# gMedAI-Lab/GAViKO

Hardware: AMD Instinct MI355X
Metric: MRI volumes/sec (fwd+bwd) ViT-B/16 gaviko, 120x160x160 (higher is better)
Workload: dtype bf16

## Files before the change

gaviko_amd/csrc/gemm_bf16.hip:

```cpp
#include "gemm_epilogue.hpp"

namespace gvk {

template <int BK>
__device__ __forceinline__ int swz_chunk(int row) {
  if constexpr (BK == 64) return (row >> 1) & 7;
  else return (0x78 >> (((row >> 2) & 3) * 2)) & 3;
}

template <int BM, int BN, int EPI, int BK = 64, bool DROP = false, int NS = 2, int NW = 4, bool SPLITK = false>
__global__ __launch_bounds__(64 * NW) void gemm_nt_kernel(GemmArgs p) {
  static_assert(NW == 4 || NW == 8, "4 or 8 waves");
  static_assert(!SPLITK || (NW == 4 && !DROP), "split-K is built on the 4-wave loops");
  static_assert(BK == 64, "the interleaved weight-row mapping is built for 128-byte tile rows");
  static_assert(NS >= 2 && NS <= 4, "2..4 LDS stages");
  constexpr int WM = BM / (NW / 2), WN = BN / 2;
  constexpr int MT = WM / 16, NT = WN / 16;
  constexpr int ROWB = BK * 2;
  constexpr int RPI = 1024 / ROWB;
  constexpr int CPR = ROWB / 16;
  constexpr int A_BYTES = BM * ROWB, W_BYTES = BN * ROWB, STAGE = A_BYTES + W_BYTES;
  extern __shared__ __attribute__((aligned(16))) char smem[];

  const int nwg = p.nbm * p.nbn;
// ... 29 lines not shown
  const bf16* __restrict__ Ag = p.A + (size_t)m0 * p.lda;
  const bf16* __restrict__ Wg = p.W + (size_t)n0 * p.ldw;
  if constexpr (SPLITK) {
    Ag += (size_t)piece * p.kt_per * BK;
    Wg += (size_t)piece * p.kt_per * BK;
  }

  auto stage = [&](int buf, int kt) {
    char* sA = smem + buf * STAGE;
    char* sW = sA + A_BYTES;
    const int k0 = kt * BK;
    const int rsub = lane / CPR, slot = lane % CPR;
#pragma unroll
    for (int r = 0; r < BM / (NW * RPI); ++r) {
      const int row = (r * NW + wave) * RPI + rsub;
      const int chunk = slot ^ swz_chunk<BK>(row);
      int srow = row;
      if constexpr (BM > 128 || 128 % BM != 0) srow = min(row, p.a_rows - 1 - m0);
      glds16(Ag + (size_t)srow * p.lda + k0 + chunk * 8, sA + (r * NW + wave) * 1024);
    }
#pragma unroll
    for (int r = 0; r < BN / (NW * RPI); ++r) {
      const int row = (r * NW + wave) * RPI + rsub;
      const int chunk = slot ^ swz_w(row);
      glds16(Wg + (size_t)row * p.ldw + k0 + chunk * 8, sW + (r * NW + wave) * 1024);
    }
  };

  f32x4 acc[MT][NT];
#pragma unroll
  for (int i = 0; i < MT; ++i)
#pragma unroll
    for (int j = 0; j < NT; ++j) acc[i][j] = f32x4{0.f, 0.f, 0.f, 0.f};

  int nt = p.K / BK;
  if constexpr (SPLITK) nt = min(p.kt_per, nt - piece * p.kt_per);
  if constexpr (BK == 64) {
#define GVK_LOAD_FRAGS(SA, SW, KS, XA, WB)                                                                  \
  {                                                                                                         \
    const int chunk_ = (KS) * 4 + lq;                                                                       \
    _Pragma("unroll") for (int i = 0; i < MT; ++i) {                                                        \
      const int row = wm * WM + i * 16 + l15;                                                               \
      XA[i] = *(const bf16x8*)((SA) + row * ROWB + ((chunk_ ^ swz_chunk<BK>(row)) << 4));                   \
    }                                                                                                       \
    _Pragma("unroll") for (int j = 0; j < NT; ++j) {                                                        \
      const int row = wn * WN + 32 * (j >> 1) + 8 * (l15 >> 2) + 4 * (j & 1) + (l15 & 3);                   \
      WB[j] = *(const bf16x8*)((SW) + row * ROWB + ((chunk_ ^ swz_w(row)) << 4));                           \
    }                                                                                                       \
  }
#define GVK_MMA(XA, WB)                                                                                      \
  _Pragma("unroll") for (int i = 0; i < MT; ++i)                                                            \
  _Pragma("unroll") for (int j = 0; j < NT; ++j)                                                            \
      acc[i][j] = __builtin_amdgcn_mfma_f32_16x16x32_bf16(WB[j], XA[i], acc[i][j], 0, 0, 0);
    bf16x8 xa0[MT], wb0[NT], xa1[MT], wb1[NT];
    constexpr int PER_TILE = BM / (NW * RPI) + BN / (NW * RPI);
    if constexpr (NS == 2) {
    stage(0, 0);
    if (nt > 1) stage(1, 1);
    if (nt > 1) __builtin_amdgcn_s_waitcnt(0x0F70 | (PER_TILE & 0xF) | ((PER_TILE >> 4) << 14));
    else __builtin_amdgcn_s_waitcnt(0x0F70);
    __builtin_amdgcn_s_barrier();
    GVK_LOAD_FRAGS(smem, smem + A_BYTES, 0, xa0, wb0)
    __builtin_amdgcn_s_waitcnt(0xC07F);
#define GVK_TILE(T, PREFETCH)                                                                               \
    {                                                                                                       \
      const int buf = (T) & 1;                                                                              \
      const char* sA = smem + buf * STAGE;                                                                  \
      const char* sW = sA + A_BYTES;                                                                        \
      GVK_LOAD_FRAGS(sA, sW, 1, xa1, wb1)                                                                   \
      __builtin_amdgcn_sched_barrier(0);                                                                    \
      GVK_MMA(xa0, wb0)                                                                                     \
      __builtin_amdgcn_sched_barrier(0);                                                                    \
      __syncthreads();     \
      if (PREFETCH) stage(buf, (T) + 2);                                                                    \
      GVK_LOAD_FRAGS(smem + (buf ^ 1) * STAGE, smem + (buf ^ 1) * STAGE + A_BYTES, 0, xa0, wb0)             \
      __builtin_amdgcn_sched_barrier(0);                                                                    \
      GVK_MMA(xa1, wb1)                                                                                     \
      __builtin_amdgcn_sched_barrier(0);                                                                    \
      __builtin_amdgcn_s_waitcnt(0xC07F);     \
    }
    int t = 0;
    for (; t < nt - 2; ++t) GVK_TILE(t, true)
    for (; t < nt; ++t) GVK_TILE(t, false)
#undef GVK_TILE
    } else {
    static_assert((NS - 1) * PER_TILE <= 63, "vmcnt is a 6-bit counter");
#pragma unroll
    for (int sgi = 0; sgi < NS; ++sgi)
      if (sgi < nt) stage(sgi, sgi);
    {
      const int ahead = min(nt, NS) - 1;
      if (ahead >= 3) __builtin_amdgcn_s_waitcnt(0x0F70 | ((3 * PER_TILE) & 0xF) | (((3 * PER_TILE) >> 4) << 14));
      else if (ahead == 2) __builtin_amdgcn_s_waitcnt(0x0F70 | ((2 * PER_TILE) & 0xF) | (((2 * PER_TILE) >> 4) << 14));
      else if (ahead == 1) __builtin_amdgcn_s_waitcnt(0x0F70 | (PER_TILE & 0xF) | ((PER_TILE >> 4) << 14));
      else __builtin_amdgcn_s_waitcnt(0x0F70);
    }
    __builtin_amdgcn_s_barrier();
    GVK_LOAD_FRAGS(smem, smem + A_BYTES, 0, xa0, wb0)
    __builtin_amdgcn_s_waitcnt(0xC07F);
#define GVK_TILE3(T, BUF, PREFETCH, AHEAD, LAST)                                                            \
    {                                                                                                       \
      const int buf = (BUF);                                                                                \
      const int nxt = buf == NS - 1 ? 0 : buf + 1;                                                          \
      const char* sA = smem + buf * STAGE;                                                                  \
      const char* sW = sA + A_BYTES;                                                                        \
      GVK_LOAD_FRAGS(sA, sW, 1, xa1, wb1)                                                                   \
      __builtin_amdgcn_sched_barrier(0);                                                                    \
      GVK_MMA(xa0, wb0)                                                                                     \
      __builtin_amdgcn_sched_barrier(0);                                                                    \
       \
      __builtin_amdgcn_s_waitcnt(0x0070 | (((AHEAD) * PER_TILE) & 0xF) | ((((AHEAD) * PER_TILE) >> 4) << 14)); \
      __builtin_amdgcn_s_barrier();                                                                         \
      if (PREFETCH) stage(buf, (T) + NS);                                                                   \
      if (!(LAST)) GVK_LOAD_FRAGS(smem + nxt * STAGE, smem + nxt * STAGE + A_BYTES, 0, xa0, wb0)            \
      __builtin_amdgcn_sched_barrier(0);                                                                    \
      GVK_MMA(xa1, wb1)                                                                                     \
      __builtin_amdgcn_sched_barrier(0);                                                                    \
      __builtin_amdgcn_s_waitcnt(0xC07F);                                                                   \
    }
    int t = 0, b = 0;
    for (; t < nt - NS; ++t) {
      GVK_TILE3(t, b, true, NS - 2, false)
      b = b == NS - 1 ? 0 : b + 1;
    }
    for (; t < nt; ++t) {
      const int r = nt - 1 - t;
      if (NS > 3 && r == 3) GVK_TILE3(t, b, false, 2, false)
      else if (r == 2) GVK_TILE3(t, b, false, 1, false)
      else if (r == 1) GVK_TILE3(t, b, false, 0, false)
      else GVK_TILE3(t, b, false, 0, true)
      b = b == NS - 1 ? 0 : b + 1;
    }
#undef GVK_TILE3
    }
#undef GVK_LOAD_FRAGS
#undef GVK_MMA
  }

  if constexpr (SPLITK) {
    const int tile_id = tile_m * p.nbn + tile_n;
    constexpr int kPiece = NW * MT * NT * 64 * 4;
    float* const base = p.sk_part + ((size_t)tile_id * p.ksplit) * kPiece;
    const __amdgpu_buffer_rsrc_t rs = __builtin_amdgcn_make_buffer_rsrc((void*)base, 0, p.ksplit * kPiece * 4, 0x00020000);
    const int off = ((wave * MT * NT) * 64 + lane) * 16;
#pragma unroll
    for (int i = 0; i < MT; ++i)
#pragma unroll
      for (int j = 0; j < NT; ++j)
        __builtin_amdgcn_raw_buffer_store_b128(__builtin_bit_cast(u32x4, acc[i][j]), rs, (piece * kPiece) * 4 + off + (i * NT + j) * 1024, 0, 16);
    int* const s_last = (int*)smem;
    asm volatile("s_waitcnt vmcnt(0)" ::: "memory");
    __syncthreads();
    if (threadIdx.x == 0) {
      const int t = __hip_atomic_fetch_add(p.sk_tick + tile_id, 1, __ATOMIC_RELAXED, __HIP_MEMORY_SCOPE_AGENT);
      const int last = (t == p.ksplit - 1) ? 1 : 0;
      if (last) {
        __builtin_amdgcn_fence(__ATOMIC_ACQUIRE, "agent");
        asm volatile("s_waitcnt vmcnt(0)" ::: "memory");
        __hip_atomic_store(p.sk_tick + tile_id, 0, __ATOMIC_RELAXED, __HIP_MEMORY_SCOPE_AGENT);
      }
      *s_last = last;
    }
    __syncthreads();
    if (!*s_last) return;
    if (p.ksplit == 2) {
      const int pc = piece ^ 1;
#pragma unroll
      for (int i = 0; i < MT; ++i)
#pragma unroll
        for (int j = 0; j < NT; ++j) acc[i][j] += *(const f32x4*)((const char*)base + (size_t)pc * kPiece * 4 + off + (i * NT + j) * 1024);
    } else {
#pragma unroll
      for (int i = 0; i < MT; ++i)
#pragma unroll
        for (int j = 0; j < NT; ++j) acc[i][j] = f32x4{0.f, 0.f, 0.f, 0.f};
      for (int pc = 0; pc < p.ksplit; ++pc) {
#pragma unroll
        for (int i = 0; i < MT; ++i)
#pragma unroll
          for (int j = 0; j < NT; ++j) acc[i][j] += *(const f32x4*)((const char*)base + (size_t)pc * kPiece * 4 + off + (i * NT + j) * 1024);
      }
    }
  }
  gemm_epilogue<EPI, DROP, MT, NT>(p, acc, m0 + wm * WM, n0 + wn * WN, l15, lq);
}

template <int BM, int BN, int EPI, bool DROP = false, int NS = 2, int NW = 4, bool SPLITK = false>
static int launch_gemm(const GemmArgs& a, hipStream_t stream) {
  constexpr int BK = 64;
  constexpr int lds = NS * (BM + BN) * BK * 2;
  static bool attr_set = false;
  if (!attr_set) {
    hipError_t e = hipFuncSetAttribute(reinterpret_cast<const void*>(&gemm_nt_kernel<BM, BN, EPI, BK, DROP, NS, NW, SPLITK>),
                                       hipFuncAttributeMaxDynamicSharedMemorySize, lds);
    if (e != hipSuccess) return set_error(-3, "hipFuncSetAttribute(gemm %dx%d): %s", BM, BN, hipGetErrorString(e));
    attr_set = true;
  }
  GemmArgs p = a;
  p.nbm = (a.M + BM - 1) / BM;
  p.nbn = a.N / BN;
  p.a_rows = (a.M + 127) / 128 * 128;
  p.m_stride = BM;
  if (a.m_stride > 0) {
    if (a.m_stride < BM || (long)(a.nbm - 1) * a.m_stride + BM > p.a_rows)
      return set_error(-2, "gvk_gemm_nt_bf16: %d row panels of %d rows at stride %d do not fit %d (padded) rows", a.nbm, BM, a.m_stride, p.a_rows);
    p.nbm = a.nbm;
    p.m_stride = a.m_stride;
  }
  {
    const int per_xcd = (p.nbm * p.nbn) >> 3;
    int g = (per_xcd + p.nbn / 2) / p.nbn;
    g = g < 1 ? 1 : g > 8 ? 8 : g;
    static const int force = diag_env("GAVIKO_HIP_GEMM_GROUP_M") ? atoi(diag_env("GAVIKO_HIP_GEMM_GROUP_M")) : 0;
    p.group_m = force > 0 ? force : g;
  }
  const int grid = p.nbm * p.nbn;
  p.xcd_panels = 0;
  {
    static const int mode = diag_env("GAVIKO_HIP_GEMM_XCD_PANELS") ? atoi(diag_env("GAVIKO_HIP_GEMM_XCD_PANELS")) : 1;
    if (mode != 0 && NS >= 3 && grid <= 256) p.xcd_panels = 1;
  }
  if constexpr (SPLITK) {
    const int nt = a.K / BK;
    int s = 256 / (grid > 0 ? grid : 1);
    s = s < 1 ? 1 : s > 8 ? 8 : s;
    if (a.ksplit > 0) s = a.ksplit;
    if (s > nt / 2) s = nt / 2 > 0 ? nt / 2 : 1;
    p.kt_per = (nt + s - 1) / s;
    p.ksplit = (nt + p.kt_per - 1) / p.kt_per;
    constexpr size_t kPiece = (size_t)NW * (BM / (NW / 2) / 16) * (BN / 2 / 16) * 64 * 4 * 4;
    const size_t need = 1024 + (size_t)grid * p.ksplit * kPiece;
    if (a.sk_part == nullptr || a.sk_bytes < need || grid > 256)
      return set_error(-2, "gvk_gemm_nt_bf16: split-K workspace of %zu bytes needed (%zu given; at most 256 tiles)", need, a.sk_bytes);
    p.sk_tick = (int*)a.sk_part;
    p.sk_part = (float*)((char*)a.sk_part + 1024);
    GVK_LAUNCH((gemm_nt_kernel<BM, BN, EPI, BK, DROP, NS, NW, SPLITK>), dim3(grid * p.ksplit), dim3(64 * NW), lds, stream, p);
    return check_launch("gemm_nt_bf16 (split-K panels)");
  }
  GVK_LAUNCH((gemm_nt_kernel<BM, BN, EPI, BK, DROP, NS, NW, SPLITK>), dim3(grid), dim3(64 * NW), lds, stream, p);
  return check_launch("gemm_nt_bf16");
}

static long wide_lo() {
  static const long v = diag_env("GAVIKO_HIP_GEMM_WIDE_LO") ? atol(diag_env("GAVIKO_HIP_GEMM_WIDE_LO")) : 140;
  return v;
}

template <int EPI>
static int dispatch_tile(const GemmArgs& a, int tile, hipStream_t stream) {
  if (a.m_stride > 0) {
    if (tile == 0) tile = (a.N % 128 == 0 && a.drop_thresh == 0u) ? 4064128 : 64064;
    if (tile == 8256256 || tile == 7256256 || tile == 256256) return set_error(-2, "gvk_gemm_nt_bf16: strided row panels run on the 4-wave tiles only");
  }
  if (tile == 0) {
    const int bn = (a.N % 128 == 0) ? 128 : 64;
    const long t128 = (long)((a.M + 127) / 128) * (a.N / bn);
    static const int n768 = diag_env("GAVIKO_HIP_GEMM_N768") ? atoi(diag_env("GAVIKO_HIP_GEMM_N768")) : 3128;
    const int bm = (t128 >= 384) ? 128 : 64;
    tile = bm * 1000 + bn;
    if constexpr (EPI == GVK_EPI_STORE_BF16 || EPI == GVK_EPI_BIAS_GELU_BF16 || EPI == GVK_EPI_GELU_BWD_BF16) {
      static const int wide = diag_env("GAVIKO_HIP_GEMM_WIDE") ? atoi(diag_env("GAVIKO_HIP_GEMM_WIDE")) : 8;
      const long t256 = (long)((a.M + 255) / 256) * (a.N / 256);
      static const bool wide_bwd = diag_env("GAVIKO_HIP_GEMM_WIDE_BWD") == nullptr || diag_env("GAVIKO_HIP_GEMM_WIDE_BWD")[0] != '0';
      if (wide != 0 && a.N % 256 == 0 && a.drop_thresh == 0u && t256 >= wide_lo() && t256 <= 256 && (EPI != GVK_EPI_GELU_BWD_BF16 || wide_bwd))
        tile = (wide == 256 || a.K < 128) ? 256256 : 8256256;
    }
    static const long t64_hi = diag_env("GAVIKO_HIP_GEMM_T64HI") ? atol(diag_env("GAVIKO_HIP_GEMM_T64HI")) : 130;
    if (bm == 64 && bn == 128 && t128 <= 256 && a.K >= 512 && a.drop_thresh == 0u) {
      if (n768 == 3128) {
        long best = -1; int best_bm = 128;
        for (int cand : {128, 96, 64}) {
          const long tiles = (long)((a.M + cand - 1) / cand) * (a.N / 128);
          const long cost = ((tiles + 255) / 256) * (cand + 128);
          if (best < 0 || cost < best) { best = cost; best_bm = cand; }
        }
        static const int force_bm = diag_env("GAVIKO_HIP_GEMM_BM") ? atoi(diag_env("GAVIKO_HIP_GEMM_BM")) : 0;
        if (force_bm == 128 || force_bm == 96 || force_bm == 64) best_bm = force_bm;
        else if (t128 <= t64_hi && best_bm == 128) best_bm = 64;
        tile = best_bm == 64 ? 3064128 : best_bm == 96 ? 3096128 : 3128128;
      }
      else if (n768 == 128) tile = 128128;
      else if (n768 == 3064) tile = 3064128;
    }
  }
  if (a.drop_thresh != 0u) {
    if constexpr (EPI == GVK_EPI_BIAS_RES_F32 || EPI == GVK_EPI_BIAS_GELU_BF16 || EPI == GVK_EPI_GELU_BWD_BF16) {
      switch (tile) {
        case 128128: return launch_gemm<128, 128, EPI, true>(a, stream);
        case 128064: return launch_gemm<128, 64, EPI, true>(a, stream);
        case 64128: return launch_gemm<64, 128, EPI, true>(a, stream);
        case 64064: return launch_gemm<64, 64, EPI, true>(a, stream);
        default: return set_error(-2, "gvk_gemm_nt_bf16: unsupported tile %d", tile);
      }
    } else {
      return set_error(-2, "gvk_gemm_nt_bf16: drop_p > 0 is supported by BIAS_RES_F32, BIAS_GELU_BF16 and GELU_BWD_BF16 only");
    }
  }
  switch (tile) {
    case 8256256: return launch_gemm8p(a, EPI, 0, stream);
    case 7256256: return launch_gemm8p(a, EPI, 1, stream);
    case 2128128:
      if (a.sk_part == nullptr) return set_error(-2, "gvk_gemm_nt_bf16: tile 2128128 needs splitk_ws");
      return launch_gemm<128, 128, EPI, false, 2, 4, true>(a, stream);
    case 3128128: return launch_gemm<128, 128, EPI, false, 3>(a, stream);
    case 3064128: return launch_gemm<64, 128, EPI, false, 3>(a, stream);
    case 4064128:
      if (a.sk_part != nullptr) return launch_gemm<64, 128, EPI, false, 4, 4, true>(a, stream);
      return launch_gemm<64, 128, EPI, false, 4>(a, stream);
    case 3096128: return launch_gemm<96, 128, EPI, false, 3>(a, stream);
    case 256256:
      if constexpr (EPI == GVK_EPI_STORE_BF16 || EPI == GVK_EPI_BIAS_GELU_BF16 || EPI == GVK_EPI_GELU_BWD_BF16) return launch_gemm<256, 256, EPI, false, 2, 8>(a, stream);
      else return set_error(-2, "gvk_gemm_nt_bf16: the 256x256 tile is built for STORE_BF16, BIAS_GELU_BF16 and GELU_BWD_BF16");
    case 128128: return launch_gemm<128, 128, EPI>(a, stream);
    case 128064: return launch_gemm<128, 64, EPI>(a, stream);
    case 64128: return launch_gemm<64, 128, EPI>(a, stream);
    case 64064: return launch_gemm<64, 64, EPI>(a, stream);
    default: return set_error(-2, "gvk_gemm_nt_bf16: unsupported tile %d", tile);
  }
}

}

extern "C" int gvk_gemm_stat_parts(int N) { return N / 64; }

extern "C" int gvk_gemm_nt_bf16(const gvk_gemm_desc* d, void* stream) {
  using namespace gvk;
  GVK_REQUIRE(d != nullptr, "gvk_gemm_nt_bf16: null descriptor");
  GVK_REQUIRE(d->a && d->w && d->M > 0 && d->N > 0 && d->K > 0, "gvk_gemm_nt_bf16: null operand or empty shape");
  GVK_REQUIRE(d->K % 64 == 0, "gvk_gemm_nt_bf16: K=%d must be a multiple of 64", d->K);
  GVK_REQUIRE(d->N % 64 == 0, "gvk_gemm_nt_bf16: N=%d must be a multiple of 64", d->N);
  GVK_REQUIRE(d->lda >= d->K && d->ldw >= d->K && d->lda % 8 == 0 && d->ldw % 8 == 0,
              "gvk_gemm_nt_bf16: lda/ldw must be >= K and multiples of 8");
  GVK_REQUIRE(d->ldo % 8 == 0 && d->ldo >= d->N, "gvk_gemm_nt_bf16: ldo=%d must be >= N and a multiple of 8 (16-byte row pieces)", d->ldo);
  if (d->tile != 0) {
    const int bn = d->tile % 1000;
    GVK_REQUIRE(d->tile < 1000000 || d->K % 32 == 0, "gvk_gemm_nt_bf16: K not a multiple of 32");
    GVK_REQUIRE(bn > 0 && d->N % bn == 0, "gvk_gemm_nt_bf16: N=%d not a multiple of the tile's BN", d->N);
  }
  GemmArgs a{};
  a.A = (const bf16*)d->a; a.W = (const bf16*)d->w; a.out0 = d->out0; a.out1 = d->out1;
  a.bias = d->bias; a.res = d->res; a.aux = (const bf16*)d->aux; a.pos = d->pos;
// ... 59 lines not shown
```

gaviko_amd/csrc/gemm8p_bf16.hip:

```cpp
#include "gemm_epilogue.hpp"

namespace gvk {

namespace {
constexpr int kUnit = 128 * 128;
constexpr int kBuf = 4 * kUnit;
constexpr int kLds = 2 * kBuf;

#define GVK_VMCNT(n) __builtin_amdgcn_s_waitcnt(0x0F70 | ((n) & 0xF) | (((n) >> 4) << 14))
#define GVK_LGKMCNT0() __builtin_amdgcn_s_waitcnt(0xC07F)

#ifdef GVK_STAMPS
#define GVK_STAMP(k) st_[k] = __builtin_amdgcn_s_memtime();
#ifndef GVK_ABLATE
#define GVK_ABLATE 0
#endif
#else
#define GVK_STAMP(k)
#define GVK_ABLATE 0
#endif
}

template <int EPI, int VAR>
__global__ __launch_bounds__(512) void gemm8p_kernel(GemmArgs p) {
// ... 94 lines not shown
  _Pragma("unroll") for (int j = 0; j < 2; ++j)                                                              \
      acc[4 * (MQ) + i][2 * (NQ) + j] =                                                                      \
          __builtin_amdgcn_mfma_f32_16x16x32_bf16(WREG[j][(C_) >> 1], xa[i][(C_) >> 1], acc[4 * (MQ) + i][2 * (NQ) + j], 0, 0, 0);

#define GVK_COMPUTE(MQ, NQ, WREG, DO_STAGE, SU, ST_, SB)                                                     \
  __builtin_amdgcn_sched_barrier(0);                                                                         \
  __builtin_amdgcn_s_barrier();                                                                              \
  if constexpr ((SB) >= 0) { GVK_STAMP((SB) < 0 ? 0 : (SB)) }                                                \
  GVK_LGKMCNT0();                                                                                            \
  if constexpr ((SB) >= 0) { GVK_STAMP((SB) < 0 ? 0 : (SB) + 1) }                                            \
  __builtin_amdgcn_sched_barrier(0);                                                                         \
  __builtin_amdgcn_s_setprio(1);                                                                             \
  GVK_MMA4(MQ, NQ, WREG, 0)                                                                                  \
  if constexpr (VAR == 1 && (DO_STAGE)) {                                                                    \
    __builtin_amdgcn_sched_barrier(0);                                                                       \
    GVK_STAGE_HALF(SU, ST_, 0)                                                                               \
    __builtin_amdgcn_sched_barrier(0);                                                                       \
  }                                                                                                          \
  GVK_MMA4(MQ, NQ, WREG, 1)                                                                                  \
  GVK_MMA4(MQ, NQ, WREG, 2)                                                                                  \
  if constexpr (VAR == 1 && (DO_STAGE)) {                                                                    \
    __builtin_amdgcn_sched_barrier(0);                                                                       \
    GVK_STAGE_HALF(SU, ST_, 1)                                                                               \
    __builtin_amdgcn_sched_barrier(0);                                                                       \
  }                                                                                                          \
  GVK_MMA4(MQ, NQ, WREG, 3)                                                                                  \
  __builtin_amdgcn_s_setprio(0);                                                                             \
  __builtin_amdgcn_sched_barrier(0);                                                                         \
  if constexpr ((SB) >= 0) { GVK_STAMP((SB) < 0 ? 0 : (SB) + 2) }                                            \
  __builtin_amdgcn_s_barrier();                                                                              \
  if constexpr ((SB) >= 0) { GVK_STAMP((SB) < 0 ? 0 : (SB) + 3) }                                            \
  __builtin_amdgcn_sched_barrier(0);

#define GVK_KTILE(T, ST, VM0, VM1, VM3, SB)                                                                      \
  {                                                                                                          \
    const int tt_ = (T);                                                                                     \
    const char* base_ = smem + (tt_ & 1) * kBuf;                                                             \
    GVK_READ_W(0, w0, base_)                                                                                 \
    GVK_READ_A(0, base_)                                                                                     \
    if constexpr (VAR == 0 && ((ST) & 1) != 0 && (GVK_ABLATE & 1) == 0) GVK_STAGE(2, tt_ + 1)                                         \
    GVK_VMCNT(VM0);                                                                                          \
    GVK_COMPUTE(0, 0, w0, ((ST) & 1) != 0, 3, tt_ + 1, SB)                                                       \
    GVK_READ_W(1, w1, base_)                                                                                 \
    if constexpr (VAR == 0 && ((ST) & 2) != 0 && (GVK_ABLATE & 1) == 0) GVK_STAGE(3, tt_ + 1)                                         \
    GVK_VMCNT(VM1);                                                                                          \
    GVK_COMPUTE(0, 1, w1, ((ST) & 2) != 0, 0, tt_ + 2, (SB) < 0 ? -1 : (SB) + 4)                                                       \
    GVK_READ_A(1, base_)                                                                                     \
    if constexpr (VAR == 0 && ((ST) & 4) != 0 && (GVK_ABLATE & 1) == 0) GVK_STAGE(0, tt_ + 2)                                         \
    GVK_COMPUTE(1, 1, w1, ((ST) & 4) != 0, 1, tt_ + 2, (SB) < 0 ? -1 : (SB) + 8)                                                       \
    if constexpr (VAR == 0 && ((ST) & 8) != 0 && (GVK_ABLATE & 1) == 0) GVK_STAGE(1, tt_ + 2)                                         \
    GVK_VMCNT(VM3);                                                                                          \
    GVK_COMPUTE(1, 0, w0, ((ST) & 8) != 0, 2, tt_ + 2, (SB) < 0 ? -1 : (SB) + 12)                                                       \
  }

  const int nt = p.K / BK;
  GVK_STAGE(0, 0) GVK_STAGE(1, 0) GVK_STAGE(2, 0) GVK_STAGE(3, 0)
  GVK_STAGE(0, 1) GVK_STAGE(1, 1)
  if constexpr (VAR == 1) {
    GVK_STAGE(2, 1)
    GVK_VMCNT(10);
  } else {
    GVK_VMCNT(8);
  }
  __builtin_amdgcn_s_barrier();
  if (wr == 1) __builtin_amdgcn_s_barrier();
  __builtin_amdgcn_sched_barrier(0);
  GVK_STAMP(1)
  int t = 0;
#ifdef GVK_STAMPS
  for (; t < nt - 3; ++t) GVK_KTILE(t, 15, 8, 8, 8, -1)
  GVK_STAMP(2)
  if (nt >= 3) { GVK_KTILE(t, 15, 8, 8, 8, 4) ++t; }
  GVK_STAMP(20)
#else
  for (; t < nt - 2; ++t) GVK_KTILE(t, 15, 8, 8, 8, -1)
#endif
  if constexpr (VAR == 1) {
    GVK_KTILE(t, 1, 8, 8, 4, -1)
    ++t;
    GVK_KTILE(t, 0, 2, 0, 63, -1)
  } else {
    GVK_KTILE(t, 3, 8, 8, 4, -1)
    ++t;
    GVK_KTILE(t, 0, 2, 0, 63, -1)
  }
  if (wr == 0) __builtin_amdgcn_s_barrier();
#undef GVK_KTILE
#undef GVK_COMPUTE
#undef GVK_MMA4
#undef GVK_STAGE_HALF
#undef GVK_READ_A
#undef GVK_READ_W
#undef GVK_STAGE

  GVK_STAMP(21)
#ifdef GVK_STAMPS
  if constexpr ((GVK_ABLATE & 2) != 0) {
#pragma unroll
    for (int i = 0; i < 4; ++i) { asm volatile("" ::"v"(xa[i][0]), "v"(xa[i][1])); }
    asm volatile("" ::"v"(w0[0][0]), "v"(w0[1][1]), "v"(w1[0][0]), "v"(w1[1][1]));
  }
  const bf16* aux_keep = p.aux;
  p.aux = nullptr;
#endif
  gemm_epilogue<EPI, false, 8, 4>(p, acc, m0 + 128 * wr, n0 + 64 * wc, l15, lq);
#ifdef GVK_STAMPS
  __builtin_amdgcn_s_waitcnt(0x0F70);
  GVK_STAMP(22)
  st_[23] = rt0_;
  st_[24] = __builtin_amdgcn_s_memrealtime();
  if (aux_keep != nullptr && lane == 0) {
    unsigned long long* o = (unsigned long long*)aux_keep + ((size_t)blockIdx.x * 8 + wave) * 32;
#pragma unroll
    for (int k = 0; k < 32; ++k) o[k] = st_[k];
  }
#endif
}

template <int EPI, int VAR>
static int launch8p(const GemmArgs& a, hipStream_t stream) {
  static bool attr_set = false;
  if (!attr_set) {
    hipError_t e = hipFuncSetAttribute(reinterpret_cast<const void*>(&gemm8p_kernel<EPI, VAR>), hipFuncAttributeMaxDynamicSharedMemorySize, kLds);
    if (e != hipSuccess) return set_error(-3, "hipFuncSetAttribute(gemm8p): %s", hipGetErrorString(e));
    attr_set = true;
  }
  GemmArgs p = a;
  p.nbm = (a.M + 255) / 256;
  p.nbn = a.N / 256;
  p.a_rows = (a.M + 127) / 128 * 128;
  GVK_LAUNCH((gemm8p_kernel<EPI, VAR>), dim3(p.nbm * p.nbn), dim3(512), kLds, stream, p);
  return check_launch("gemm8p_bf16");
}

bool gemm8p_supports(int epilogue) {
  switch (epilogue) {
    case GVK_EPI_STORE_BF16: case GVK_EPI_BIAS_GELU_BF16: case GVK_EPI_GELU_BWD_BF16: case GVK_EPI_STORE_F32: case GVK_EPI_BIAS_RES_F32:
      return true;
// ... 25 lines not shown
```

gaviko_amd/csrc/gemm_epilogue.hpp:

```cpp
#pragma once
#include "common.hpp"
#include "dropout.hpp"
#include "../../include/gaviko_hip.h"

namespace gvk {

struct GemmArgs {
  const bf16* A;
  const bf16* W;
  void* out0;
  void* out1;
  const float* bias;
  const float* res;
  const bf16* aux;
  const float* pos;
  int M, N, K, lda, ldw, ldo, ldres, ldaux;
  int rows_in, rows_out, row_off;
  int nbm, nbn;
  int group_m;
  int xcd_panels;
  int a_rows;
  int m_stride;
  int ksplit, kt_per;
  float* sk_part;
  int* sk_tick;
  size_t sk_bytes;
  unsigned long long seed; const unsigned long long* seed_ptr; unsigned int drop_thresh; float inv_keep;
  int scale_cols; float col_scale;
  const float* ln_mean; const float* ln_rstd; const float* ln_c1;
  float* stat_part;
  const float* stat_pivot;
  int aux_grad;
};

__device__ __forceinline__ int swz_a128(int row) { return (row >> 1) & 7; }
__device__ __forceinline__ int swz_w(int row) { return ((row >> 1) & 1) | (((row >> 3) & 3) << 1); }

template <int EPI, bool DROP, int MT, int NT>
__device__ __forceinline__ void gemm_epilogue(const GemmArgs& p, f32x4 (&acc)[MT][NT], const int mbase, const int nbase, const int l15, const int lq) {
  static_assert(NT % 2 == 0, "tile pairs");
  constexpr int NP = NT / 2;
  constexpr bool kRes = EPI == GVK_EPI_BIAS_RES_F32 || EPI == GVK_EPI_BIAS_RES_F32_BF16;
  constexpr bool kAux = EPI == GVK_EPI_GELU_BWD_BF16 || EPI == GVK_EPI_RELU_BWD_BF16;
  constexpr bool kPos = EPI == GVK_EPI_PATCH_F32;
  constexpr bool kFold = EPI == GVK_EPI_STORE_BF16;
  constexpr bool kStat = EPI == GVK_EPI_BIAS_RES_F32_BF16;
  f32x4 bv[NP][2];
  [[maybe_unused]] f32x4 c1v[NP][2];
#pragma unroll
  for (int jp = 0; jp < NP; ++jp) {
    bv[jp][0] = bv[jp][1] = f32x4{0.f, 0.f, 0.f, 0.f};
    const int n = nbase + 32 * jp + 8 * lq;
    if (p.bias != nullptr) {
      bv[jp][0] = *(const f32x4*)(p.bias + n);
      bv[jp][1] = *(const f32x4*)(p.bias + n + 4);
    }
    if constexpr (kFold) {
      c1v[jp][0] = c1v[jp][1] = f32x4{0.f, 0.f, 0.f, 0.f};
      if (p.ln_mean != nullptr) {
        c1v[jp][0] = *(const f32x4*)(p.ln_c1 + n);
        c1v[jp][1] = *(const f32x4*)(p.ln_c1 + n + 4);
      }
    }
  }
  struct Side { f32x4 r0[NP], r1[NP]; bf16x8 a8[NP]; float mu, rs, pv; };
  auto fetch = [&](const int i, Side& sd) {
    const int m = mbase + i * 16 + l15;
    if (m >= p.M) return;
    if constexpr (kFold) {
      if (p.ln_mean != nullptr) { sd.mu = p.ln_mean[m]; sd.rs = p.ln_rstd[m]; }
    }
    if constexpr (kStat) sd.pv = p.stat_pivot != nullptr ? p.stat_pivot[m] : 0.f;
#pragma unroll
    for (int jp = 0; jp < NP; ++jp) {
      const int n = nbase + 32 * jp + 8 * lq;
      if constexpr (kRes) {
        const float* rp = p.res + (size_t)m * p.ldres + n;
        sd.r0[jp] = *(const f32x4*)rp;
        sd.r1[jp] = *(const f32x4*)(rp + 4);
      } else if constexpr (kPos) {
        const float* pp = p.pos + (size_t)(m % p.rows_in) * p.N + n;
        sd.r0[jp] = *(const f32x4*)pp;
        sd.r1[jp] = *(const f32x4*)(pp + 4);
      } else if constexpr (kAux) {
        sd.a8[jp] = *(const bf16x8*)(p.aux + (size_t)m * p.ldaux + n);
      }
    }
  };
  Side cur, nxt;
  fetch(0, cur);
#pragma unroll
  for (int i = 0; i < MT; ++i) {
    if (i + 1 < MT) fetch(i + 1, nxt);
    const int m = mbase + i * 16 + l15;
    [[maybe_unused]] float ps1 = 0.f, ps2 = 0.f;
    if (m < p.M) {
      size_t orow = (size_t)m;
      if constexpr (kPos) {
        const int s = m / p.rows_in;
        orow = (size_t)s * p.rows_out + p.row_off + (m - s * p.rows_in);
      }
#pragma unroll
      for (int jp = 0; jp < NP; ++jp) {
        const int n = nbase + 32 * jp + 8 * lq;
        float v[8];
#pragma unroll
        for (int e = 0; e < 4; ++e) { v[e] = acc[i][2 * jp][e] + bv[jp][0][e]; v[4 + e] = acc[i][2 * jp + 1][e] + bv[jp][1][e]; }
        if constexpr (kFold) {
          if (p.ln_mean != nullptr) {
#pragma unroll
            for (int e = 0; e < 4; ++e) {
              v[e] = __builtin_fmaf(__builtin_fmaf(-cur.mu, c1v[jp][0][e], acc[i][2 * jp][e]), cur.rs, bv[jp][0][e]);
              v[4 + e] = __builtin_fmaf(__builtin_fmaf(-cur.mu, c1v[jp][1][e], acc[i][2 * jp + 1][e]), cur.rs, bv[jp][1][e]);
            }
          }
        }
        auto store_f32 = [&](float* dst) {
          *(f32x4*)dst = f32x4{v[0], v[1], v[2], v[3]};
          *(f32x4*)(dst + 4) = f32x4{v[4], v[5], v[6], v[7]};
        };
        auto store_bf16 = [&](bf16* dst) {
          bf16x8 o;
#pragma unroll
          for (int e = 0; e < 8; ++e) o[e] = (bf16)v[e];
          *(bf16x8*)dst = o;
        };
// ... 78 lines not shown
```

Before: 767.9.

## Add deep-pipelined 64-row panel GEMM kernel for strided row-panel launches

Result: no change. 768.2, median of 3 (+0.0%).

```diff
diff --git a/gaviko_amd/csrc/gemm_bf16.hip b/gaviko_amd/csrc/gemm_bf16.hip
--- a/gaviko_amd/csrc/gemm_bf16.hip
+++ b/gaviko_amd/csrc/gemm_bf16.hip
@@ -238,6 +238,162 @@
   gemm_epilogue<EPI, DROP, MT, NT>(p, acc, m0 + wm * WM, n0 + wn * WN, l15, lq);
 }
 
+template <int N>
+__device__ __forceinline__ void wait_vm_lgkm0() {
+  static_assert(N >= 0 && N <= 63, "vmcnt is a 6-bit counter");
+  __builtin_amdgcn_s_waitcnt(0x0070 | (N & 0xF) | ((N >> 4) << 14));
+}
+
+template <int PER, int MAXT>
+__device__ __forceinline__ void wait_tiles_lgkm0(const int tiles) {
+  if constexpr (MAXT > 0) {
+    if (tiles >= MAXT) wait_vm_lgkm0<PER * MAXT>();
+    else wait_tiles_lgkm0<PER, MAXT - 1>(tiles);
+  } else {
+    wait_vm_lgkm0<0>();
+  }
+}
+
+template <int EPI, int NS, int BN>
+__global__ __launch_bounds__(256) void gemm_panel_kernel(GemmArgs p) {
+  static_assert(BN == 64 || BN == 32, "64 or 32 columns");
+  static_assert(NS >= 3 && NS <= 10, "3..10 LDS stages (160 KiB)");
+  constexpr int BM = 64, BK = 64, NW = 4;
+  constexpr int WAVES_N = BN / 32, WAVES_M = NW / WAVES_N;
+  constexpr int WM = BM / WAVES_M, WN = 32;
+  constexpr int MT = WM / 16, NT = WN / 16;
+  constexpr int ROWB = BK * 2, RPI = 1024 / ROWB, CPR = ROWB / 16;
+  constexpr int A_BYTES = BM * ROWB, W_BYTES = BN * ROWB, STAGE = A_BYTES + W_BYTES;
+  constexpr int A_PER = BM / (NW * RPI), W_PER = BN / (NW * RPI), PER_TILE = A_PER + W_PER;
+  static_assert((NS - 1) * PER_TILE <= 63, "vmcnt is a 6-bit counter");
+  extern __shared__ __attribute__((aligned(16))) char smem[];
+
+  const int nwg = p.nbm * p.nbn;
+  const int bid = blockIdx.x, xcd = bid & 7, q = nwg >> 3, r = nwg & 7;
+  const int wg = (xcd < r ? xcd * (q + 1) : r * (q + 1) + (xcd - r) * q) + (bid >> 3);
+  const int tile_n = wg / p.nbm, tile_m = wg - tile_n * p.nbm;
+  const int m0 = tile_m * p.m_stride, n0 = tile_n * BN;
+
+  const int lane = lane_id();
+  const int wave = wave_id();
+  const int wm = wave / WAVES_N, wn = wave % WAVES_N;
+  const int l15 = lane & 15, lq = lane >> 4;
+  const int nt = p.K / BK;
+
+  const bf16* asrc[A_PER];
+  const bf16* wsrc[W_PER];
+  {
+    const int rsub = lane / CPR, slot = lane % CPR;
+#pragma unroll
+    for (int i = 0; i < A_PER; ++i) {
+      const int row = (i * NW + wave) * RPI + rsub;
+      asrc[i] = p.A + (size_t)(m0 + row) * p.lda + (slot ^ swz_chunk<BK>(row)) * 8;
+    }
+#pragma unroll
+    for (int i = 0; i < W_PER; ++i) {
+      const int row = (i * NW + wave) * RPI + rsub;
+      wsrc[i] = p.W + (size_t)(n0 + row) * p.ldw + (slot ^ swz_w(row)) * 8;
+    }
+  }
+  auto stage = [&](int buf, int kt) {
+    char* sA = smem + buf * STAGE;
+    char* sW = sA + A_BYTES;
+    const int k0 = min(kt, nt - 1) * BK;
+#pragma unroll
+    for (int i = 0; i < A_PER; ++i) glds16(asrc[i] + k0, sA + (i * NW + wave) * 1024);
+#pragma unroll
+    for (int i = 0; i < W_PER; ++i) glds16(wsrc[i] + k0, sW + (i * NW + wave) * 1024);
+  };
+#pragma unroll
+  for (int s = 0; s < NS; ++s) stage(s, s);
+
+  f32x4 acc[MT][NT];
+#pragma unroll
+  for (int i = 0; i < MT; ++i)
+#pragma unroll
+    for (int j = 0; j < NT; ++j) acc[i][j] = f32x4{0.f, 0.f, 0.f, 0.f};
+
+#define GVK_LOAD_FRAGS(SA, SW, KS, XA, WB)                                                                  \
+  {                                                                                                         \
+    const int chunk_ = (KS) * 4 + lq;                                                                       \
+    _Pragma("unroll") for (int i = 0; i < MT; ++i) {                                                        \
+      const int row = wm * WM + i * 16 + l15;                                                               \
+      XA[i] = *(const bf16x8*)((SA) + row * ROWB + ((chunk_ ^ swz_chunk<BK>(row)) << 4));                   \
+    }                                                                                                       \
+    _Pragma("unroll") for (int j = 0; j < NT; ++j) {                                                        \
+      const int row = wn * WN + 32 * (j >> 1) + 8 * (l15 >> 2) + 4 * (j & 1) + (l15 & 3);                   \
+      WB[j] = *(const bf16x8*)((SW) + row * ROWB + ((chunk_ ^ swz_w(row)) << 4));                           \
+    }                                                                                                       \
+  }
+#define GVK_MMA(XA, WB)                                                                                      \
+  _Pragma("unroll") for (int i = 0; i < MT; ++i)                                                            \
+  _Pragma("unroll") for (int j = 0; j < NT; ++j)                                                            \
+      acc[i][j] = __builtin_amdgcn_mfma_f32_16x16x32_bf16(WB[j], XA[i], acc[i][j], 0, 0, 0);
+#define GVK_PANEL_TILE(T, BUF, WAIT, PREFETCH, LAST)                                                        \
+  {                                                                                                         \
+    const int buf = (BUF);                                                                                  \
+    const int nxt = buf == NS - 1 ? 0 : buf + 1;                                                            \
+    const char* sA = smem + buf * STAGE;                                                                    \
+    GVK_LOAD_FRAGS(sA, sA + A_BYTES, 1, xa1, wb1)                                                           \
+    __builtin_amdgcn_sched_barrier(0);                                                                      \
+    GVK_MMA(xa0, wb0)                                                                                       \
+    __builtin_amdgcn_sched_barrier(0);                                                                      \
+    WAIT;                                                                                                   \
+    __builtin_amdgcn_s_barrier();                                                                           \
+    if (PREFETCH) stage(buf, (T) + NS);                                                                     \
+    if (!(LAST)) GVK_LOAD_FRAGS(smem + nxt * STAGE, smem + nxt * STAGE + A_BYTES, 0, xa0, wb0)              \
+    __builtin_amdgcn_sched_barrier(0);                                                                      \
+    GVK_MMA(xa1, wb1)                                                                                       \
+    __builtin_amdgcn_sched_barrier(0);                                                                      \
+    __builtin_amdgcn_s_waitcnt(0xC07F);           \
+  }
+  bf16x8 xa0[MT], wb0[NT], xa1[MT], wb1[NT];
+  wait_vm_lgkm0<(NS - 1) * PER_TILE>();
+  __builtin_amdgcn_s_barrier();
+  GVK_LOAD_FRAGS(smem, smem + A_BYTES, 0, xa0, wb0)
+  __builtin_amdgcn_s_waitcnt(0xC07F);
+  int t = 0, b = 0;
+  for (; t < nt - NS; ++t) {
+    GVK_PANEL_TILE(t, b, wait_vm_lgkm0<(NS - 2) * PER_TILE>(), true, false)
+    b = b == NS - 1 ? 0 : b + 1;
+  }
+  for (; t < nt - 1; ++t) {
+    const int after = max(nt, NS) - t - 2;
+    GVK_PANEL_TILE(t, b, (wait_tiles_lgkm0<PER_TILE, NS - 2>(after)), false, false)
+    b = b == NS - 1 ? 0 : b + 1;
+  }
+  GVK_PANEL_TILE(t, b, wait_vm_lgkm0<0>(), false, true)
+#undef GVK_PANEL_TILE
+#undef GVK_LOAD_FRAGS
+#undef GVK_MMA
+  gemm_epilogue<EPI, false, MT, NT>(p, acc, m0 + wm * WM, n0 + wn * WN, l15, lq);
+}
+
+template <int EPI, int NS, int BN>
+static int launch_panel(const GemmArgs& a, hipStream_t stream) {
+  constexpr int lds = NS * (64 + BN) * 128;
+  static bool attr_set = false;
+  if (!attr_set) {
+    hipError_t e = hipFuncSetAttribute(reinterpret_cast<const void*>(&gemm_panel_kernel<EPI, NS, BN>), hipFuncAttributeMaxDynamicSharedMemorySize, lds);
+    if (e != hipSuccess) return set_error(-3, "hipFuncSetAttribute(panel gemm %d x 64x%d): %s", NS, BN, hipGetErrorString(e));
+    attr_set = true;
+  }
+  GemmArgs p = a;
+  p.a_rows = (a.M + 127) / 128 * 128;
+  if (a.m_stride < 64 || (long)(a.nbm - 1) * a.m_stride + 64 > p.a_rows)
+    return set_error(-2, "gvk_gemm_nt_bf16: %d row panels of %d rows at stride %d do not fit %d (padded) rows", a.nbm, 64, a.m_stride, p.a_rows);
+  p.nbn = a.N / BN;
+  GVK_LAUNCH((gemm_panel_kernel<EPI, NS, BN>), dim3(p.nbm * p.nbn), dim3(256), lds, stream, p);
+  return check_launch("gemm_nt_bf16 (row panels)");
+}
+
+template <int EPI>
+static bool panel_form_takes(const GemmArgs& a) {
+  constexpr bool epi = EPI == GVK_EPI_BIAS_GELU_BF16 || EPI == GVK_EPI_BIAS_RES_F32 || EPI == GVK_EPI_GELU_BWD_BF16 || EPI == GVK_EPI_STORE_BF16 ||
+                       EPI == GVK_EPI_STORE_F32;
+  return epi && a.m_stride > 0 && a.sk_part == nullptr && a.drop_thresh == 0u && a.ln_mean == nullptr && a.stat_part == nullptr;
+}
+
 template <int BM, int BN, int EPI, bool DROP = false, int NS = 2, int NW = 4, bool SPLITK = false>
 static int launch_gemm(const GemmArgs& a, hipStream_t stream) {
   constexpr int BK = 64;
@@ -299,9 +455,12 @@
   return v;
 }
 
+static int panel_tile(const GemmArgs& a) { return (long)a.nbm * (a.N / 32) <= 256 ? 8064032 : 8064064; }
+
 template <int EPI>
 static int dispatch_tile(const GemmArgs& a, int tile, hipStream_t stream) {
   if (a.m_stride > 0) {
+    if (tile == 0 && panel_form_takes<EPI>(a)) tile = panel_tile(a);
     if (tile == 0) tile = (a.N % 128 == 0 && a.drop_thresh == 0u) ? 4064128 : 64064;
     if (tile == 8256256 || tile == 7256256 || tile == 256256) return set_error(-2, "gvk_gemm_nt_bf16: strided row panels run on the 4-wave tiles only");
   }
@@ -360,6 +519,13 @@
     case 4064128:
       if (a.sk_part != nullptr) return launch_gemm<64, 128, EPI, false, 4, 4, true>(a, stream);
       return launch_gemm<64, 128, EPI, false, 4>(a, stream);
+    case 8064064: case 8064032:
+      if constexpr (EPI == GVK_EPI_BIAS_GELU_BF16 || EPI == GVK_EPI_BIAS_RES_F32 || EPI == GVK_EPI_GELU_BWD_BF16 || EPI == GVK_EPI_STORE_BF16 || EPI == GVK_EPI_STORE_F32) {
+        if (!panel_form_takes<EPI>(a)) return set_error(-2, "gvk_gemm_nt_bf16: tile %d is the row-panel form (m_panels, no splitk_ws / dropout / LayerNorm fold)", tile);
+        return tile == 8064064 ? launch_panel<EPI, 8, 64>(a, stream) : launch_panel<EPI, 8, 32>(a, stream);
+      } else {
+        return set_error(-2, "gvk_gemm_nt_bf16: tile %d is built for the five epilogues of the pruned launches", tile);
+      }
     case 3096128: return launch_gemm<96, 128, EPI, false, 3>(a, stream);
     case 256256:
       if constexpr (EPI == GVK_EPI_STORE_BF16 || EPI == GVK_EPI_BIAS_GELU_BF16 || EPI == GVK_EPI_GELU_BWD_BF16) return launch_gemm<256, 256, EPI, false, 2, 8>(a, stream);
```

## Prefetch epilogue side operands during final K-tiles of GEMM mainloop

Applied to the files above, without the earlier changes.

Measured after the change: 774.3 before, 783.2 after (median of 6 runs). 1.1% higher.

```diff
diff --git a/gaviko_amd/csrc/gemm8p_bf16.hip b/gaviko_amd/csrc/gemm8p_bf16.hip
--- a/gaviko_amd/csrc/gemm8p_bf16.hip
+++ b/gaviko_amd/csrc/gemm8p_bf16.hip
@@ -150,7 +150,7 @@
   if constexpr ((SB) >= 0) { GVK_STAMP((SB) < 0 ? 0 : (SB) + 3) }                                            \
   __builtin_amdgcn_sched_barrier(0);
 
-#define GVK_KTILE(T, ST, VM0, VM1, VM3, SB)                                                                      \
+#define GVK_KTILE(T, ST, VM0, VM1, VM3, SB, SIDE)                                                                 \
   {                                                                                                          \
     const int tt_ = (T);                                                                                     \
     const char* base_ = smem + (tt_ & 1) * kBuf;                                                             \
@@ -164,6 +164,7 @@
     GVK_VMCNT(VM1);                                                                                          \
     GVK_COMPUTE(0, 1, w1, ((ST) & 2) != 0, 0, tt_ + 2, (SB) < 0 ? -1 : (SB) + 4)                                                       \
     GVK_READ_A(1, base_)                                                                                     \
+    if constexpr (SIDE) pre.issue(p, m0 + 128 * wr, n0 + 64 * wc, l15, lq);                                  \
     if constexpr (VAR == 0 && ((ST) & 4) != 0 && (GVK_ABLATE & 1) == 0) GVK_STAGE(0, tt_ + 2)                                         \
     GVK_COMPUTE(1, 1, w1, ((ST) & 4) != 0, 1, tt_ + 2, (SB) < 0 ? -1 : (SB) + 8)                                                       \
     if constexpr (VAR == 0 && ((ST) & 8) != 0 && (GVK_ABLATE & 1) == 0) GVK_STAGE(1, tt_ + 2)                                         \
@@ -171,6 +172,13 @@
     GVK_COMPUTE(1, 0, w0, ((ST) & 8) != 0, 2, tt_ + 2, (SB) < 0 ? -1 : (SB) + 12)                                                       \
   }
 
+#ifdef GVK_STAMPS
+  constexpr int PF = 0;
+#else
+  constexpr int PF = EPI == GVK_EPI_GELU_BWD_BF16 ? 3 : EPI == GVK_EPI_BIAS_RES_F32 ? 1 : 0;
+#endif
+  EpiPrefetch<EPI, 4, PF> pre;
+  constexpr int NPRE = PF > 0 ? EpiPrefetch<EPI, 4, PF>::kLoads : 0;
   const int nt = p.K / BK;
   GVK_STAGE(0, 0) GVK_STAGE(1, 0) GVK_STAGE(2, 0) GVK_STAGE(3, 0)
   GVK_STAGE(0, 1) GVK_STAGE(1, 1)
@@ -186,21 +194,21 @@
   GVK_STAMP(1)
   int t = 0;
 #ifdef GVK_STAMPS
-  for (; t < nt - 3; ++t) GVK_KTILE(t, 15, 8, 8, 8, -1)
+  for (; t < nt - 3; ++t) GVK_KTILE(t, 15, 8, 8, 8, -1, false)
   GVK_STAMP(2)
-  if (nt >= 3) { GVK_KTILE(t, 15, 8, 8, 8, 4) ++t; }
+  if (nt >= 3) { GVK_KTILE(t, 15, 8, 8, 8, 4, false) ++t; }
   GVK_STAMP(20)
 #else
-  for (; t < nt - 2; ++t) GVK_KTILE(t, 15, 8, 8, 8, -1)
+  for (; t < nt - 2; ++t) GVK_KTILE(t, 15, 8, 8, 8, -1, false)
 #endif
   if constexpr (VAR == 1) {
-    GVK_KTILE(t, 1, 8, 8, 4, -1)
+    GVK_KTILE(t, 1, 8, 8, 4 + NPRE, -1, PF > 0)
     ++t;
-    GVK_KTILE(t, 0, 2, 0, 63, -1)
+    GVK_KTILE(t, 0, 2 + NPRE, NPRE, 63, -1, false)
   } else {
-    GVK_KTILE(t, 3, 8, 8, 4, -1)
+    GVK_KTILE(t, 3, 8, 8, 4 + NPRE, -1, PF > 0)
     ++t;
-    GVK_KTILE(t, 0, 2, 0, 63, -1)
+    GVK_KTILE(t, 0, 2 + NPRE, NPRE, 63, -1, false)
   }
   if (wr == 0) __builtin_amdgcn_s_barrier();
 #undef GVK_KTILE
@@ -221,7 +229,7 @@
   const bf16* aux_keep = p.aux;
   p.aux = nullptr;
 #endif
-  gemm_epilogue<EPI, false, 8, 4>(p, acc, m0 + 128 * wr, n0 + 64 * wc, l15, lq);
+  gemm_epilogue<EPI, false, 8, 4, PF>(p, acc, m0 + 128 * wr, n0 + 64 * wc, l15, lq, pre);
 #ifdef GVK_STAMPS
   __builtin_amdgcn_s_waitcnt(0x0F70);
   GVK_STAMP(22)
diff --git a/gaviko_amd/csrc/gemm_bf16.hip b/gaviko_amd/csrc/gemm_bf16.hip
--- a/gaviko_amd/csrc/gemm_bf16.hip
+++ b/gaviko_amd/csrc/gemm_bf16.hip
@@ -85,6 +85,10 @@
   for (int i = 0; i < MT; ++i)
 #pragma unroll
     for (int j = 0; j < NT; ++j) acc[i][j] = f32x4{0.f, 0.f, 0.f, 0.f};
+
+  constexpr int PF = (NS >= 3 && !DROP && !SPLITK && kEpiSideOperand<EPI>) ? MT : 0;
+  EpiPrefetch<EPI, NT, PF> pre;
+  constexpr int NPRE = PF > 0 ? EpiPrefetch<EPI, NT, PF>::kLoads : 0;
 
   int nt = p.K / BK;
   if constexpr (SPLITK) nt = min(p.kt_per, nt - piece * p.kt_per);
@@ -137,21 +141,25 @@
     for (; t < nt; ++t) GVK_TILE(t, false)
 #undef GVK_TILE
     } else {
-    static_assert((NS - 1) * PER_TILE <= 63, "vmcnt is a 6-bit counter");
+    static_assert((NS - 1) * PER_TILE <= 63 && (NS - 2) * PER_TILE + NPRE <= 63, "vmcnt is a 6-bit counter");
 #pragma unroll
     for (int sgi = 0; sgi < NS; ++sgi)
       if (sgi < nt) stage(sgi, sgi);
+    const bool pre_early = PF > 0 && nt < NS;
+    if (pre_early) pre.issue(p, m0 + wm * WM, n0 + wn * WN, l15, lq);
+#define GVK_VMCNT_(N_) __builtin_amdgcn_s_waitcnt(0x0F70 | ((N_) & 0xF) | (((N_) >> 4) << 14))
     {
       const int ahead = min(nt, NS) - 1;
-      if (ahead >= 3) __builtin_amdgcn_s_waitcnt(0x0F70 | ((3 * PER_TILE) & 0xF) | (((3 * PER_TILE) >> 4) << 14));
-      else if (ahead == 2) __builtin_amdgcn_s_waitcnt(0x0F70 | ((2 * PER_TILE) & 0xF) | (((2 * PER_TILE) >> 4) << 14));
-      else if (ahead == 1) __builtin_amdgcn_s_waitcnt(0x0F70 | (PER_TILE & 0xF) | ((PER_TILE >> 4) << 14));
-      else __builtin_amdgcn_s_waitcnt(0x0F70);
-    }
+      if (ahead >= 3) GVK_VMCNT_(3 * PER_TILE);
+      else if (ahead == 2) { if (pre_early) GVK_VMCNT_(2 * PER_TILE + NPRE); else GVK_VMCNT_(2 * PER_TILE); }
+      else if (ahead == 1) { if (pre_early) GVK_VMCNT_(PER_TILE + NPRE); else GVK_VMCNT_(PER_TILE); }
+      else { if (pre_early) GVK_VMCNT_(NPRE); else GVK_VMCNT_(0); }
+    }
+#undef GVK_VMCNT_
     __builtin_amdgcn_s_barrier();
     GVK_LOAD_FRAGS(smem, smem + A_BYTES, 0, xa0, wb0)
     __builtin_amdgcn_s_waitcnt(0xC07F);
-#define GVK_TILE3(T, BUF, PREFETCH, AHEAD, LAST)                                                            \
+#define GVK_TILE3(T, BUF, PREFETCH, AHEAD, LAST, SIDE, XV)                                                  \
     {                                                                                                       \
       const int buf = (BUF);                                                                                \
       const int nxt = buf == NS - 1 ? 0 : buf + 1;                                                          \
@@ -162,9 +170,10 @@
       GVK_MMA(xa0, wb0)                                                                                     \
       __builtin_amdgcn_sched_barrier(0);                                                                    \
        \
-      __builtin_amdgcn_s_waitcnt(0x0070 | (((AHEAD) * PER_TILE) & 0xF) | ((((AHEAD) * PER_TILE) >> 4) << 14)); \
+      __builtin_amdgcn_s_waitcnt(0x0070 | (((AHEAD) * PER_TILE + (XV)) & 0xF) | ((((AHEAD) * PER_TILE + (XV)) >> 4) << 14)); \
       __builtin_amdgcn_s_barrier();                                                                         \
       if (PREFETCH) stage(buf, (T) + NS);                                                                   \
+      if constexpr (SIDE) pre.issue(p, m0 + wm * WM, n0 + wn * WN, l15, lq);                                \
       if (!(LAST)) GVK_LOAD_FRAGS(smem + nxt * STAGE, smem + nxt * STAGE + A_BYTES, 0, xa0, wb0)            \
       __builtin_amdgcn_sched_barrier(0);                                                                    \
       GVK_MMA(xa1, wb1)                                                                                     \
@@ -172,17 +181,36 @@
       __builtin_amdgcn_s_waitcnt(0xC07F);                                                                   \
     }
     int t = 0, b = 0;
-    for (; t < nt - NS; ++t) {
-      GVK_TILE3(t, b, true, NS - 2, false)
-      b = b == NS - 1 ? 0 : b + 1;
-    }
-    for (; t < nt; ++t) {
-      const int r = nt - 1 - t;
-      if (NS > 3 && r == 3) GVK_TILE3(t, b, false, 2, false)
-      else if (r == 2) GVK_TILE3(t, b, false, 1, false)
-      else if (r == 1) GVK_TILE3(t, b, false, 0, false)
-      else GVK_TILE3(t, b, false, 0, true)
-      b = b == NS - 1 ? 0 : b + 1;
+    if (PF == 0 || nt >= NS) {
+      for (; t < nt - NS; ++t) {
+        GVK_TILE3(t, b, true, NS - 2, false, false, 0)
+        b = b == NS - 1 ? 0 : b + 1;
+      }
+    }
+    if constexpr (PF == 0) {
+      for (; t < nt; ++t) {
+        const int r = nt - 1 - t;
+        if (NS > 3 && r == 3) GVK_TILE3(t, b, false, 2, false, false, 0)
+        else if (r == 2) GVK_TILE3(t, b, false, 1, false, false, 0)
+        else if (r == 1) GVK_TILE3(t, b, false, 0, false, false, 0)
+        else GVK_TILE3(t, b, false, 0, true, false, 0)
+        b = b == NS - 1 ? 0 : b + 1;
+      }
+    } else if (nt >= NS) {
+#define GVK_NEXT_BUF b = b == NS - 1 ? 0 : b + 1; ++t;
+      if constexpr (NS > 3) { GVK_TILE3(t, b, false, 2, false, true, 0) GVK_NEXT_BUF }
+      GVK_TILE3(t, b, false, 1, false, NS == 3, NS == 3 ? 0 : NPRE) GVK_NEXT_BUF
+      GVK_TILE3(t, b, false, 0, false, false, NPRE) GVK_NEXT_BUF
+      GVK_TILE3(t, b, false, 0, true, false, NPRE)
+#undef GVK_NEXT_BUF
+    } else {
+      for (; t < nt; ++t) {
+        const int r = nt - 1 - t;
+        if (r == 2) GVK_TILE3(t, b, false, 1, false, false, NPRE)
+        else if (r == 1) GVK_TILE3(t, b, false, 0, false, false, NPRE)
+        else GVK_TILE3(t, b, false, 0, true, false, NPRE)
+        b = b == NS - 1 ? 0 : b + 1;
+      }
     }
 #undef GVK_TILE3
     }
@@ -235,7 +263,7 @@
       }
     }
   }
-  gemm_epilogue<EPI, DROP, MT, NT>(p, acc, m0 + wm * WM, n0 + wn * WN, l15, lq);
+  gemm_epilogue<EPI, DROP, MT, NT, PF>(p, acc, m0 + wm * WM, n0 + wn * WN, l15, lq, pre);
 }
 
 template <int BM, int BN, int EPI, bool DROP = false, int NS = 2, int NW = 4, bool SPLITK = false>
diff --git a/gaviko_amd/csrc/gemm_epilogue.hpp b/gaviko_amd/csrc/gemm_epilogue.hpp
--- a/gaviko_amd/csrc/gemm_epilogue.hpp
+++ b/gaviko_amd/csrc/gemm_epilogue.hpp
@@ -36,8 +36,48 @@
 __device__ __forceinline__ int swz_a128(int row) { return (row >> 1) & 7; }
 __device__ __forceinline__ int swz_w(int row) { return ((row >> 1) & 1) | (((row >> 3) & 3) << 1); }
 
-template <int EPI, bool DROP, int MT, int NT>
-__device__ __forceinline__ void gemm_epilogue(const GemmArgs& p, f32x4 (&acc)[MT][NT], const int mbase, const int nbase, const int l15, const int lq) {
+template <int EPI>
+constexpr bool kEpiSideOperand = EPI == GVK_EPI_BIAS_RES_F32 || EPI == GVK_EPI_BIAS_RES_F32_BF16 || EPI == GVK_EPI_GELU_BWD_BF16;
+
+template <int EPI, int NT, int PF>
+struct EpiPrefetch {
+  static constexpr int NP = NT / 2;
+  static constexpr bool kRes = EPI == GVK_EPI_BIAS_RES_F32 || EPI == GVK_EPI_BIAS_RES_F32_BF16;
+  static constexpr bool kStat = EPI == GVK_EPI_BIAS_RES_F32_BF16;
+  static constexpr int kLoads = PF * (NP * (kRes ? 2 : 1) + (kStat ? 1 : 0));
+  u32x4 q[PF > 0 ? PF : 1][NP][2];
+  float pv[PF > 0 ? PF : 1];
+
+  __device__ __forceinline__ void issue(const GemmArgs& p, const int mbase, const int nbase, const int l15, const int lq) {
+    if constexpr (PF > 0) {
+      constexpr int ES = kRes ? 4 : 2;
+      const int ld = kRes ? p.ldres : p.ldaux;
+      const int live = __builtin_amdgcn_readfirstlane(min(p.M - mbase, 16 * PF));
+      const char* base = (kRes ? (const char*)p.res : (const char*)p.aux) + ((size_t)mbase * ld + nbase) * ES;
+      const unsigned bytes = live > 0 ? (unsigned)(((live - 1) * ld + 16 * NT) * ES) : 0u;
+      const __amdgpu_buffer_rsrc_t rs = __builtin_amdgcn_make_buffer_rsrc((void*)base, 0, bytes, 0x00020000);
+#pragma unroll
+      for (int i = 0; i < PF; ++i)
+#pragma unroll
+        for (int jp = 0; jp < NP; ++jp) {
+          const int off = ((i * 16 + l15) * ld + 32 * jp + 8 * lq) * ES;
+          q[i][jp][0] = __builtin_amdgcn_raw_buffer_load_b128(rs, off, 0, 0);
+          if constexpr (kRes) q[i][jp][1] = __builtin_amdgcn_raw_buffer_load_b128(rs, off + 16, 0, 0);
+        }
+      if constexpr (kStat) {
+        const __amdgpu_buffer_rsrc_t rp =
+            __builtin_amdgcn_make_buffer_rsrc((void*)(p.stat_pivot + mbase), 0, (p.stat_pivot != nullptr && live > 0) ? (unsigned)live * 4u : 0u, 0x00020000);
+#pragma unroll
+        for (int i = 0; i < PF; ++i) pv[i] = __builtin_bit_cast(float, __builtin_amdgcn_raw_buffer_load_b32(rp, (i * 16 + l15) * 4, 0, 0));
+      }
+    }
+  }
+};
+
+template <int EPI, bool DROP, int MT, int NT, int PF = 0>
+__device__ __forceinline__ void gemm_epilogue(const GemmArgs& p, f32x4 (&acc)[MT][NT], const int mbase, const int nbase, const int l15, const int lq,
+                                              const EpiPrefetch<EPI, NT, PF>& pre = EpiPrefetch<EPI, NT, PF>{}) {
+  static_assert(PF == 0 || (kEpiSideOperand<EPI> && PF <= MT), "prefetched row groups: side-operand epilogues only");
   static_assert(NT % 2 == 0, "tile pairs");
   constexpr int NP = NT / 2;
   constexpr bool kRes = EPI == GVK_EPI_BIAS_RES_F32 || EPI == GVK_EPI_BIAS_RES_F32_BF16;
@@ -88,10 +128,23 @@
     }
   };
   Side cur, nxt;
-  fetch(0, cur);
+  if constexpr (PF == 0) fetch(0, cur);
+  else __builtin_amdgcn_s_waitcnt(0x0F70);
 #pragma unroll
   for (int i = 0; i < MT; ++i) {
-    if (i + 1 < MT) fetch(i + 1, nxt);
+    if (i + 1 < MT && i + 1 >= PF) fetch(i + 1, nxt);
+    if (i < PF) {
+      if constexpr (kStat) cur.pv = pre.pv[i];
+#pragma unroll
+      for (int jp = 0; jp < NP; ++jp) {
+        if constexpr (kRes) {
+          cur.r0[jp] = __builtin_bit_cast(f32x4, pre.q[i][jp][0]);
+          cur.r1[jp] = __builtin_bit_cast(f32x4, pre.q[i][jp][1]);
+        } else if constexpr (kAux) {
+          cur.a8[jp] = __builtin_bit_cast(bf16x8, pre.q[i][jp][0]);
+        }
+      }
+    }
     const int m = mbase + i * 16 + l15;
     [[maybe_unused]] float ps1 = 0.f, ps2 = 0.f;
     if (m < p.M) {
```
